# tqch/v-diffusion-torch

Measured on AMD Instinct MI355X. Metric: train_images_per_sec, higher is better.
Workload: dtype fp32 (bf16x3 split products in the tile-engine GEMMs)

## Files before the change

v-diffusion-torch_amd/csrc/norm.hip:

```cpp
#include "common.h"
#include <stdlib.h>

namespace {

constexpr int PPC = 128;

template <bool NT>
__device__ __forceinline__ f32x4 ld_stream(const float* p) {
    if (NT) return __builtin_nontemporal_load(reinterpret_cast<const f32x4*>(p));
    return *reinterpret_cast<const f32x4*>(p);
}
template <bool NT>
__device__ __forceinline__ void st_stream(float* p, f32x4 v) {
    if (NT) __builtin_nontemporal_store(v, reinterpret_cast<f32x4*>(p));
    else *reinterpret_cast<f32x4*>(p) = v;
}

struct ReduceArgs {
    const float* x; long long ldx;
    const float* dy; long long lddy;
    const float* coef;
    int act; float p_drop; unsigned long long seed; int resample; int has_norm;
    int H, W;
    long long HW;
    int C, nimg, chunks;
    float* part;
};

__device__ __forceinline__ f32x4 dz_finish(const ReduceArgs& p, f32x4 g, f32x4 xv, f32x4 sc, f32x4 of, unsigned long long vec_index) {
    if (p.p_drop > 0.f) g *= vd_dropout_scale4(p.seed, vec_index, p.p_drop);
    if (p.act) {
#pragma unroll
        for (int j = 0; j < 4; ++j) {
            const float z = xv[j] * sc[j] + of[j];
            const float s = vd_sigmoid(z);
            g[j] *= s * (1.f + z * (1.f - s));
        }
    }
    return g;
}

__device__ __forceinline__ f32x4 dz_of(const ReduceArgs& p, const float* dy_img, int pix, int c4, f32x4 xv, f32x4 sc,
                                       f32x4 of, unsigned long long vec_index) {
    f32x4 g;
    if (p.resample == VD_RS_NONE) {
        g = *reinterpret_cast<const f32x4*>(dy_img + (long long)pix * p.lddy + c4);
    } else {
        const int y = pix / p.W, x = pix - y * p.W;
        if (p.resample == VD_RS_DOWN) {
            const int Wo = p.W >> 1;
            g = *reinterpret_cast<const f32x4*>(dy_img + ((long long)(y >> 1) * Wo + (x >> 1)) * p.lddy + c4) * 0.25f;
        } else {
            const int Wo = p.W << 1;
            const float* b0 = dy_img + ((long long)(2 * y) * Wo + 2 * x) * p.lddy + c4;
            g = *reinterpret_cast<const f32x4*>(b0) + *reinterpret_cast<const f32x4*>(b0 + p.lddy) +
// ... 355 lines not shown
    const int c = (int)((long long)blockIdx.x - it[7]) * 16 + cx;
    float a = 0.f, bsum = 0.f;
    if (c < C)
        for (int b = ly; b < nimg; b += 16) { a += pgb[((long long)b * 2) * C + c]; bsum += pgb[((long long)b * 2 + 1) * C + c]; }
    sh[0][ly][cx] = a; sh[1][ly][cx] = bsum;
    __syncthreads();
    if (ly == 0 && c < C) {
        float s0 = 0.f, s1 = 0.f;
#pragma unroll
        for (int q = 0; q < 16; ++q) { s0 += sh[0][q][cx]; s1 += sh[1][q][cx]; }
        dgamma[c] = accumulate ? dgamma[c] + s0 : s0;
        dbeta[c] = accumulate ? dbeta[c] + s1 : s1;
    }
}

struct BwdApplyArgs {
    ReduceArgs r; const float* q; const float* add; long long ldadd; float* dx; long long lddx; int accumulate_dx;
};

__global__ __launch_bounds__(256) void gn_bwd_apply_kernel(const BwdApplyArgs a, int Cb) {
    const ReduceArgs& p = a.r;
    const int b = blockIdx.y, c0 = blockIdx.z * Cb;
    const int vecs = min(Cb, p.C - c0) >> 2, rows = 256 / vecs;
    const int r = threadIdx.x / vecs, c4 = c0 + 4 * (threadIdx.x % vecs);
    if (r >= rows) return;
    const int HW = (int)p.HW;
    const int p0 = blockIdx.x * APIX, np = min(APIX, HW - p0);
    f32x4 sc = {1.f, 1.f, 1.f, 1.f}, of = {0.f, 0.f, 0.f, 0.f}, nr = sc, nm = of;
    f32x4 q0 = sc, q1 = of, q2 = of;
    if (p.has_norm) {
        const float* cf = p.coef + (long long)b * 4 * p.C;
        sc = *reinterpret_cast<const f32x4*>(cf + c4);
        of = *reinterpret_cast<const f32x4*>(cf + p.C + c4);
        nr = *reinterpret_cast<const f32x4*>(cf + 2 * p.C + c4);
// ... 37 lines not shown
    for (int i = r; i < np; i += rows) {
        const int pix = p0 + i;
        f32x4 xv = {0.f, 0.f, 0.f, 0.f};
        if (p.has_norm) xv = *reinterpret_cast<const f32x4*>(ximg + (long long)pix * p.ldx + c4);
        const unsigned long long vi = ((unsigned long long)b * p.HW + pix) * vtot + (c4 >> 2);
        f32x4 d = dz_of(p, dimg, pix, c4, xv, sc, of, vi);
        if (p.has_norm) d = q0 * d - q1 - (xv * nr + nm) * q2;
        if (aimg) d += *reinterpret_cast<const f32x4*>(aimg + (long long)pix * a.ldadd + c4);
        float* o = oimg + (long long)pix * a.lddx + c4;
        if (a.accumulate_dx) d += *reinterpret_cast<const f32x4*>(o);
        *reinterpret_cast<f32x4*>(o) = d;
    }
}


struct FusedBwdArgs {
    BwdApplyArgs a; const float* gamma; const float* beta; const float* film; float* dfilm; float* pgb; int G, CS;
    int nsplit; float* xbuf; unsigned* cnt;
    unsigned* spin_max;
};

template <int NPT, int TPB, bool NT = false, bool SPLIT = false>
__global__ __launch_bounds__(TPB) void gn_bwd_fused_kernel(const FusedBwdArgs f) {
    __shared__ float red[TPB][8];
    __shared__ float chs[2][128];
    __shared__ float gm[2][32];
    constexpr int NREG = (NPT == 8 && TPB == 1024) ? 4 : NPT;
    __shared__ f32x4 xl[NPT - NREG > 0 ? NPT - NREG : 1][NPT - NREG > 0 ? TPB : 1];
    const ReduceArgs& p = f.a.r;
    const int CS = f.CS, C = p.C, tid = threadIdx.x;
    int b = blockIdx.y, slab = blockIdx.x, sib = 0, unit = 0;
    if (SPLIT) {
        const int lid = blockIdx.x, q = lid >> 3;
        sib = q % f.nsplit;
        unit = (q / f.nsplit) * 8 + (lid & 7);
        const int nslab = C / CS;
// ... 98 lines not shown
            }
            if (VD_PROBE_BUILD && f.spin_max) atomicMax(f.spin_max, spin);
        }
        __syncthreads();
        if (tid < 2 * CS) {
            const float* all = f.xbuf + (long long)unit * f.nsplit * 256 + (tid / CS) * 128 + (tid % CS);
            float t = 0.f;
            for (int k = 0; k < f.nsplit; ++k) t += __hip_atomic_load(all + k * 256, __ATOMIC_RELAXED, __HIP_MEMORY_SCOPE_AGENT);
            if (__hip_atomic_load(f.cnt + unit, __ATOMIC_RELAXED, __HIP_MEMORY_SCOPE_AGENT) >= (1u << 20)) t = __builtin_nanf("");
            chs[tid / CS][tid % CS] = t;
        }
        __syncthreads();
    }
    const int cg = C / f.G;
    if (tid < CS) {
        const int c = c0 + tid;
        const float s1 = chs[0][tid], s2 = chs[1][tid];
        float fs = 1.f;
        if (f.film) {
            fs = 1.f + f.film[(long long)b * 2 * C + C + c];
            if (sib == 0) {
                f.dfilm[(long long)b * 2 * C + c] = s1;
                f.dfilm[(long long)b * 2 * C + C + c] = f.gamma[c] * s2 + f.beta[c] * s1;
            }
        }
        const float k = f.gamma[c] * fs;
        if (sib == 0) {
            f.pgb[((long long)b * 2) * C + c] = fs * s2;
            f.pgb[((long long)b * 2 + 1) * C + c] = fs * s1;
        }
        chs[0][tid] = k * s1; chs[1][tid] = k * s2;
    }
    __syncthreads();
    if (tid < CS / cg) {
        float m1 = 0.f, m2 = 0.f;
        for (int c = tid * cg; c < (tid + 1) * cg; ++c) { m1 += chs[0][c]; m2 += chs[1][c]; }
        const float inv = 1.f / ((float)cg * (float)p.HW);
        gm[0][tid] = m1 * inv; gm[1][tid] = m2 * inv;
    }
    __syncthreads();
    if (!act) return;
    f32x4 q0, q1, q2;
#pragma unroll
    for (int j = 0; j < 4; ++j) {
        const int cl = 4 * v + j, c = c0 + cl, g = cl / cg;
        const float fs = f.film ? 1.f + f.film[(long long)b * 2 * C + C + c] : 1.f;
        q0[j] = nr[j] * f.gamma[c] * fs; q1[j] = nr[j] * gm[0][g]; q2[j] = nr[j] * gm[1][g];
    }
    const float* aimg = f.a.add ? f.a.add + ((long long)b * p.HW + pbeg) * f.a.ldadd : nullptr;
    float* oimg = f.a.dx + ((long long)b * p.HW + pbeg) * f.a.lddx;
#pragma unroll
    for (int i = 0; i < NPT; ++i) {
        const f32x4 xh = i < NREG ? xv[i < NREG ? i : 0] : xl[i < NREG ? 0 : i - NREG][tid];
        dz[i] = q0 * dz[i] - q1 - xh * q2;
    }
    if (aimg) {
        f32x4 ad[NPT];
#pragma unroll
        for (int i = 0; i < NPT; ++i) ad[i] = *reinterpret_cast<const f32x4*>(aimg + (long long)min(r + i * rows, HW - 1) * f.a.ldadd + c4);
#pragma unroll
        for (int i = 0; i < NPT; ++i) dz[i] += ad[i];
    }
    if (f.a.accumulate_dx) {
        f32x4 od[NPT];
#pragma unroll
        for (int i = 0; i < NPT; ++i) od[i] = *reinterpret_cast<const f32x4*>(oimg + (long long)min(r + i * rows, HW - 1) * f.a.lddx + c4);
#pragma unroll
        for (int i = 0; i < NPT; ++i) dz[i] += od[i];
    }
// ... 318 lines not shown
```

v-diffusion-torch_amd/csrc/wino43.hip:

```cpp
#include "common.h"
#include "../../include/vdiff_hip_dgrad_planes.h"
#include <stdlib.h>
#include <type_traits>

namespace {

typedef __attribute__((address_space(3))) void* lds_ptr_t;
constexpr unsigned OOB = 0x80000000u;
constexpr int KT = 8;
constexpr int TN = 32;
constexpr int TILES = 64;
constexpr int U_STAGE = 36 * 4 * 16 * 2 * 2;
constexpr int THREADS = 512;

struct Args43 {
    const float* x; long long ldx;
    const float* U;
    float* y; long long ldy;
    int nimg, H, W, K, N;
    int items_per_img;
    int ngrp;
    int ncb, nitems;
    const float* bias; const float* res; long long ldr;
    float* stats;
// ... 755 lines not shown
    o[0] = 1.265625f * v[0];
    o[1] = 1.6875f * q12 + 0.84375f * q34 + 1.265625f * v[5];
    o[2] = -2.8125f * v[0] - 2.25f * p12 - 0.5625f * p34;
    o[3] = -0.75f * q12 - 1.5f * q34 - 2.8125f * v[5];
    o[4] = v[0] + p12 + p34;
    o[5] = v[5];
}

struct In43 {
    const float* dV; long long plane;
    float* dx; long long lddx;
    int Cin;
};

template <int TW>
__global__ __launch_bounds__(256) void wino43_in_transpose_kernel(const In43 p) {
    constexpr int TPI = TW * TW, NQ = 256 / TPI;
    __shared__ f32x4 ring[12][256];
    const int tid = threadIdx.x, q = tid % NQ, tile = tid / NQ;
    const int ty = tile / TW, tx = tile - ty * TW;
    const int c4 = ((int)blockIdx.x * NQ + q) * 4;
    const bool in = c4 < p.Cin;
    f32x4 S[6][4];
    if (in) {
        const float* vp = p.dV + ((long long)blockIdx.y * TPI + tile) * p.Cin + c4;
#pragma unroll
        for (int a = 0; a < 6; ++a) {
            f32x4 v[6], r[6];
#pragma unroll
            for (int b = 0; b < 6; ++b) v[b] = *reinterpret_cast<const f32x4*>(vp + (long long)(6 * a + b) * p.plane);
            b6(v, r);
            ring[a][tid] = r[0]; ring[6 + a][tid] = r[5];
#pragma unroll
            for (int c = 0; c < 4; ++c) S[a][c] = r[c + 1];
        }
    }
    __syncthreads();
    if (in) {
        if (tx > 0) {
#pragma unroll
            for (int a = 0; a < 6; ++a) S[a][0] += ring[6 + a][tid - NQ];
        }
        if (tx < TW - 1) {
#pragma unroll
            for (int a = 0; a < 6; ++a) S[a][3] += ring[a][tid + NQ];
        }
    }
    __syncthreads();
    f32x4 P[4][4];
    if (in) {
#pragma unroll
        for (int c = 0; c < 4; ++c) {
            const f32x4 col[6] = {S[0][c], S[1][c], S[2][c], S[3][c], S[4][c], S[5][c]};
            f32x4 o[6];
            b6(col, o);
            ring[c][tid] = o[0]; ring[4 + c][tid] = o[5];
#pragma unroll
            for (int u = 0; u < 4; ++u) P[u][c] = o[u + 1];
        }
    }
    __syncthreads();
    if (!in) return;
    if (ty > 0) {
#pragma unroll
        for (int c = 0; c < 4; ++c) P[0][c] += ring[4 + c][tid - TW * NQ];
    }
    if (ty < TW - 1) {
#pragma unroll
        for (int c = 0; c < 4; ++c) P[3][c] += ring[c][tid + TW * NQ];
    }
    float* xp = p.dx + (((long long)blockIdx.y * (4 * TW) + 4 * ty) * (4 * TW) + 4 * tx) * p.lddx + c4;
#pragma unroll
    for (int u = 0; u < 4; ++u)
#pragma unroll
        for (int c = 0; c < 4; ++c) *reinterpret_cast<f32x4*>(xp + (long long)(u * 4 * TW + c) * p.lddx) = P[u][c];
}

struct Wg43Plan { bool ok; int T, S; size_t v_f, m_f, u_f, cs_f, gemm_bytes; };
Wg43Plan wg43_plan(int nimg, int H, int W, int Cin, int Cout) {
    Wg43Plan g = {};
    if (nimg <= 0 || H % 4 || W % 4 || H < 4 || W < 4 || Cin % 4 || Cout % 4) return g;
    g.T = nimg * (H / 4) * (W / 4);
    g.S = vd_gemm_grouped_wgrad_auto_split(36, Cout, Cin, g.T, (g.T + 1535) / 1536, 24);
    const size_t T16 = ((size_t)g.T + 15) / 16 * 16;
    g.v_f = (size_t)36 * T16 * Cin; g.m_f = (size_t)36 * T16 * Cout; g.u_f = (size_t)36 * Cout * Cin; g.cs_f = (size_t)36 * Cout;
    g.gemm_bytes = vd_gemm_grouped_wgrad_ws_bytes(36, Cout, Cin, g.S);
    g.ok = true;
    return g;
}

// ... 339 lines not shown
    return 1;
}

extern "C" size_t vd_conv3x3_wino43_dgrad_planes_ws_bytes(int32_t nimg, int32_t H, int32_t W, int32_t Cin, int32_t Cout) {
    const size_t T = (size_t)nimg * (H / 4) * (W / 4);
    return ((size_t)36 * Cout * Cin + (size_t)36 * T * Cin) * sizeof(float);
}

extern "C" int vd_conv3x3_dgrad_planes_preferred(int32_t nimg, int32_t H, int32_t W, int32_t Cin, int32_t Cout, int32_t training) {
    if (!training || !vd_conv3x3_wino43_dgrad_planes_supported(nimg, H, W, Cin, Cout, Cin)) return 0;
    static const long long floor_t = getenv("VD_PLANES_MIN_TILES") ? atoll(getenv("VD_PLANES_MIN_TILES")) : VD_PLANES_MIN_TILES;
    const long long T = (long long)nimg * (H / 4) * (W / 4);
    return T >= floor_t && Cin % 256 == 0 && Cout % 16 == 0;
}

extern "C" int vd_conv3x3_wino43_dgrad_planes(const float* dM, const float* w_oihw, float* dx, int64_t lddx, int32_t nimg, int32_t H, int32_t W,
                                              int32_t Cin, int32_t Cout, float* ws, size_t ws_bytes, int32_t phase, void* stream) {
    VD_REQUIRE(dM && w_oihw && dx && ws, "vd_conv3x3_wino43_dgrad_planes: null operand");
    VD_REQUIRE(vd_conv3x3_wino43_dgrad_planes_supported(nimg, H, W, Cin, Cout, lddx),
               "vd_conv3x3_wino43_dgrad_planes: unsupported geometry nimg=%d H=%d W=%d Cin=%d Cout=%d", nimg, H, W, Cin, Cout);
    VD_REQUIRE(vd_aligned16(dM) && vd_aligned16(dx) && vd_aligned16(ws), "vd_conv3x3_wino43_dgrad_planes: operands must be 16-byte aligned");
    VD_REQUIRE(ws_bytes >= vd_conv3x3_wino43_dgrad_planes_ws_bytes(nimg, H, W, Cin, Cout), "vd_conv3x3_wino43_dgrad_planes: workspace too small");
    VD_REQUIRE(phase == 7 || phase == 1 || phase == 2 || phase == 4, "vd_conv3x3_wino43_dgrad_planes: phase must be 7, 1, 2 or 4");
    const int TPI = (H / 4) * (W / 4), T = nimg * TPI;
    float* Ut = ws;
    float* dV = ws + (size_t)36 * Cout * Cin;
    hipStream_t st = (hipStream_t)stream;
    if (phase & 1) {
        const long long plane = (long long)Cout * Cin;
        hipLaunchKernelGGL(wino43_pack_planes_t_kernel, dim3((unsigned)((plane + 255) / 256)), dim3(256), 0, st, w_oihw, Ut, Cout, Cin);
        VD_LAUNCH_CHECK("wino43_pack_planes_t_kernel");
    }
    if (phase & 2) {
        vd_gemm_desc d = {};
        d.A = dM; d.B = Ut; d.C = dV;
        d.M = T; d.N = Cin; d.K = Cout; d.a_kind = VD_ROW; d.b_kind = VD_ROW;
        d.lda = Cout; d.ldb = Cout; d.ldc = Cin;
        d.batch = 36; d.nh = 1; d.alpha = 1.f;
        d.sAb = 16LL * Cout; d.sBb = (long long)Cout * Cin; d.sCb = (long long)T * Cin;
        const int rc = vd_gemm_rowblk(&d, 36LL * 16 * Cout, stream);
        if (rc) return rc;
    }
    if (phase & 4) {
        In43 o = {};
        o.dV = dV; o.plane = (long long)T * Cin; o.dx = dx; o.lddx = lddx; o.Cin = Cin;
        if (W == 32)
            hipLaunchKernelGGL(wino43_in_transpose_kernel<8>, dim3((unsigned)((Cin + 15) / 16), (unsigned)nimg), dim3(256), 0, st, o);
        else
            hipLaunchKernelGGL(wino43_in_transpose_kernel<4>, dim3((unsigned)((Cin + 63) / 64), (unsigned)nimg), dim3(256), 0, st, o);
        VD_LAUNCH_CHECK("wino43_in_transpose_kernel");
    }
    return 0;
}
```

v-diffusion-torch_amd/v_diffusion/_hip.py:

```python
import ctypes as C
import os
import re

import numpy as np
import torch

_HERE = os.path.dirname(os.path.abspath(__file__))
HEADER_PATH = os.path.join(os.path.dirname(os.path.dirname(_HERE)), "include", "vdiff_hip.h")
LIB_PATH = os.environ.get("VDIFF_HIP_LIB") or os.path.join(os.path.dirname(_HERE), "lib", "libvdiff_hip.so")

ROW, COL, IM2COL = 0, 1, 2
TILE_WIDE = 128256
RS_NONE, RS_DOWN, RS_UP = 0, 1, 2
OUT_TYPES = {"v": 0, "x0": 1, "eps": 2, "both": 3}
REWEIGHTS = {"constant": 0, "snr": 1, "snr_trunc": 2, "snr_1plus": 3}

_i32, _i64, _f32, _vp = C.c_int32, C.c_int64, C.c_float, C.c_void_p


class GemmDesc(C.Structure):
    _fields_ = [("A", _vp), ("B", _vp), ("C", _vp), ("bias", _vp), ("R", _vp),
                ("M", _i32), ("N", _i32), ("K", _i32), ("a_kind", _i32), ("b_kind", _i32),
                ("lda", _i64), ("ldb", _i64), ("ldc", _i64), ("ldr", _i64),
                ("batch", _i32), ("nh", _i32),
# ... 43 lines not shown
    if not os.path.exists(path):
        raise RuntimeError(f"{path} not found: the ctypes binding is read from the C headers of the source tree")
    with open(path) as f:
        tables = _parse_header(f.read())
    return [{name: _ctypes_of(name, *decl) for name, decl in t.items()} for t in tables]


_SIGNATURES, PROBE_EXPORTS = _header_signatures()
EXPORTS = tuple(_SIGNATURES)
EXT_HEADER_PATHS = (os.path.join(os.path.dirname(HEADER_PATH), "vdiff_hip_dgrad_planes.h"),)
_EXT_SIGNATURES = {name: sig for path in EXT_HEADER_PATHS for name, sig in _header_signatures(path)[0].items()}
EXT_EXPORTS = tuple(_EXT_SIGNATURES)
DPS_HEADER_PATHS = (os.path.join(os.path.dirname(HEADER_PATH), "vdiff_hip_dps.h"),)
_DPS_SIGNATURES = {name: sig for path in DPS_HEADER_PATHS for name, sig in _header_signatures(path)[0].items()}
DPS_EXPORTS = tuple(_DPS_SIGNATURES)

_lib = None


def lib():
    global _lib
    if _lib is None:
        if not os.path.exists(LIB_PATH):
            raise RuntimeError(
                f"{LIB_PATH} not found: build it with `python __graft_entry__.py` (or make -C v-diffusion-torch_amd/csrc). "
                "The v_diffusion hot path has no CPU/PyTorch fallback.")
        l = C.CDLL(LIB_PATH)
        for name, (res, args) in {**_SIGNATURES, **_EXT_SIGNATURES, **_DPS_SIGNATURES}.items():
            fn = getattr(l, name)
            fn.restype, fn.argtypes = res, args
        for name, (res, args) in PROBE_EXPORTS.items():
            if hasattr(l, name):
                fn = getattr(l, name)
                fn.restype, fn.argtypes = res, args
        _lib = l
    return _lib


class HipError(RuntimeError):
    pass


_CPU_TENSOR = "v_diffusion HIP op received a CPU tensor: the hot path runs on an MI355X only (no CPU fallback)"
# ... 344 lines not shown
def conv3x3_wino43_dgrad_planes(dm, w, dx, lddx, nimg, H, W, Cin, Cout):
    assert dm.numel() >= lib().vd_conv3x3_wino43_dm_floats(nimg, H, W, Cout) and w.is_contiguous() and tuple(w.shape) == (Cout, Cin, 3, 3)
    ws = workspace(lib().vd_conv3x3_wino43_dgrad_planes_ws_bytes(nimg, H, W, Cin, Cout), dm.device, "dgrad_planes")
    args = (ptr(dm), ptr(w), ptr(dx), lddx, nimg, H, W, Cin, Cout, ws.data_ptr(), ws.numel() * 4)
    phase = lambda ph: _check(lib().vd_conv3x3_wino43_dgrad_planes(*args, ph, stream()), "vd_conv3x3_wino43_dgrad_planes")
    if PROFILE is None:
        phase(7)
        return
    T = nimg * (H // 4) * (W // 4)
    with _TimedBytes("wino43_pack_planes_t_kernel", 4.0 * (9 + 36) * Cout * Cin):
        phase(1)
    with _TimedTile("gemm_dma_kernel<{tile}, 0, 0, false, {kt}>", 2.0 * 36 * T * Cout * Cin):
        phase(2)
    _note_bytes(PROFILE[-1][0], 4.0 * 36.0 * (T * (Cin + Cout) + Cout * Cin))
    with _TimedBytes("wino43_in_transpose_kernel", 4.0 * (36.0 * T * Cin + nimg * H * W * Cin)):
        phase(4)


def conv3x3_dgrad_wino43(dy, lddy, U43, dx, lddx, nimg, H, W, Cin, Cout):
    with _TimedName(f"wino43_conv_kernel<{W // 4}, false>", 2.0 * nimg * H * W * Cout * 9 * Cin):
        _check(lib().vd_conv3x3_dgrad_wino43(ptr(dy), lddy, ptr(U43), ptr(dx), lddx, nimg, H, W, Cin, Cout, stream()),
               "vd_conv3x3_dgrad_wino43")
    _note_bytes(f"wino43_conv_kernel<{W // 4}, false>", 4.0 * (nimg * H * W * (Cin + Cout) + 36 * Cout * Cin))


def conv3x3(x, ldx, wpack, bias, y, ldy, nimg, H, W, Cin, Cout, res=None, ldres=0, accumulate=False, stats_part=None):
    with _TimedTile("gemm_dma_kernel<{tile}, 2, 0, false, {kt}>", 2.0 * nimg * H * W * Cout * 9 * Cin):
        _check(lib().vd_conv3x3(ptr(x), ldx, ptr(wpack), ptr(bias), ptr(res), ldres, ptr(y), ldy, nimg, H, W, Cin, Cout,
                                int(accumulate), ptr(stats_part), stream()), "vd_conv3x3")

# ... 579 lines not shown
```

v-diffusion-torch_amd/v_diffusion/engine.py:

```python
import collections
import contextlib
import math

import torch

from . import _hip as H

GROUPS = 32
EPS = 1e-6
THIN = 8


def _ld(t):
    return t.stride(2)


def _chk(t):
    B, Hh, Ww, C = t.shape
    ld = t.stride(2)
    assert t.stride(3) == 1 and t.stride(1) == Ww * ld and t.stride(0) == Hh * Ww * ld, "not an NHWC view"
    return B, Hh, Ww, C, ld


def _splitk(M, N, K, n=1):
# ... 233 lines not shown
        if len(q) == H.GROUP_MAX:
            self._wgrad_flush_key(key)

    def _cwgrad(self, x, ldx, dy, lddy, *args, v=None, **kw):
        if v is not None:
            kw["v"] = v
        side = self._side
        if side is None:
            return H.conv3x3_wgrad(x, ldx, dy, lddy, *args, **kw)
        side.wait_stream(torch.cuda.current_stream())
        (x if v is None else v).record_stream(side)
        dy.record_stream(side)
        with torch.cuda.stream(side):
            H.conv3x3_wgrad(x, ldx, dy, lddy, *args, **kw)

    def _conv_bwd_planes(self, w, v, dy, lddy, dx, lddx, B, Hh, Ww, Cin, Cout, gw, gb):
        if v is None or not H.dgrad_planes_supported(B, Hh, Ww, Cin, Cout, lddy, lddx):
            return False
        dm = torch.empty(H.lib().vd_conv3x3_wino43_dm_floats(B, Hh, Ww, Cout), dtype=torch.float32, device=dy.device)
        H.conv3x3_wino43_dy_image(dy, lddy, B, Hh, Ww, Cout, dm)
        side = self._side
        if gw is None:
            pass
        elif side is None:
            H.conv3x3_wgrad_wino43_vm(v, dm, B, Hh, Ww, Cin, Cout, gw, Cin, Cout, dbias=gb)
        else:
            side.wait_stream(torch.cuda.current_stream())
            v.record_stream(side)
            dm.record_stream(side)
            with torch.cuda.stream(side):
                H.conv3x3_wgrad_wino43_vm(v, dm, B, Hh, Ww, Cin, Cout, gw, Cin, Cout, dbias=gb)
        H.conv3x3_wino43_dgrad_planes(dm, w, dx, lddx, B, Hh, Ww, Cin, Cout)
        return True

    def _side_join(self):
        if self._side is not None:
            torch.cuda.current_stream().wait_stream(self._side)

    def _wgrad_flush_key(self, key):
        q = self._wq.pop(key, None)
        if not q:
            return
        M, N, K, lda, ldb, ldc, _ = key
        ok = M % 4 == 0 and N % 4 == 0 and lda % 4 == 0 and ldb % 4 == 0 and max(lda, ldb, ldc) * 128 + 128 < 0x70000000 // 4 and \
            all(dy.data_ptr() % 16 == 0 and x.data_ptr() % 16 == 0 for dy, x, _, _ in q)
        if len(q) == 1 or not ok:
            for dy, x, dw, db in q:
# ... 282 lines not shown
                          ldres=_ld(sk), stats_part=pd, keep_v=v2)
        out_parts = self._parts(pd, Cout, Ho * Wo, rows)
        if tape is not None:
            tape[prefix] = dict(x=x, coef1=coef1, a1=None if v1 else a1, h1=h1, coef2=coef2, a2=None if v2 else a2, film=film,
                                xs=xs if has_skip else None, seed=seed, p=p_drop, v1=v1[0] if v1 else None, v2=v2[0] if v2 else None)
        return out_parts

    def _res_bwd(self, blk, ctx, dy, dx, dx_accumulate, ta, dfilms, G):
        mod = blk.res
        only_dx = G is None
        g = _NO_GRADS if only_dx else {s: G[name] for s, name in blk.res_names.items()}
        x, a1, h1, a2, film = ctx["x"], ctx["a1"], ctx["h1"], ctx["a2"], ctx["film"]
        B, Hh, Ww, Cin, ldx = _chk(x)
        _, Ho, Wo, Cout, lddy = _chk(dy)
        rs = blk.rs
        da2 = self._new(x, B, Ho, Wo, Cout)
        if not self._conv_bwd_planes(mod.conv2.weight, ctx["v2"], dy, lddy, da2, Cout, B, Ho, Wo, Cout, Cout, g["conv2.weight"], g["conv2.bias"]):
            if not only_dx:
                self._cwgrad(a2, Cout, dy, lddy, B, Ho, Wo, Cout, Cout, g["conv2.weight"], Cout, Cout, dbias=g["conv2.bias"], v=ctx["v2"])
            self._conv(dy, lddy, mod.conv2.weight, None, da2, Cout, B, Ho, Wo, Cout, Cout, dgrad=True)
        dh1 = self._new(x, B, Ho, Wo, Cout)
        c2, fi = blk.film
        dfilm = dfilms[c2][0 if only_dx else fi]
        H.gn_apply_bwd(da2, Cout, h1, Cout, ctx["coef2"], mod.norm2.weight, mod.norm2.bias, film, 1, ctx["p"], ctx["seed"],
                       H.RS_NONE, None, 0, dh1, Cout, False, dfilm, None, None, False, B, Ho, Wo, Cout, GROUPS,
                       pgb_keep=self._pgb(B, Cout, g["norm2.weight"], g["norm2.bias"]))
        del da2
        da1 = self._new(x, B, Ho, Wo, Cin)
        if not self._conv_bwd_planes(mod.conv1.weight, ctx["v1"], dh1, Cout, da1, Cin, B, Ho, Wo, Cin, Cout, g["conv1.weight"], g["conv1.bias"]):
            if not only_dx:
                self._cwgrad(a1, Cin, dh1, Cout, B, Ho, Wo, Cin, Cout, g["conv1.weight"], Cin, Cout, dbias=g["conv1.bias"], v=ctx["v1"])
            self._conv(dh1, Cout, mod.conv1.weight, None, da1, Cin, B, Ho, Wo, Cout, Cin, dgrad=True)
        del dh1
        if Cin != Cout:
            xs = ctx["xs"]
            P = B * Ho * Wo
            w = mod.skip.weight
            if not only_dx:
                self._wgrad(dy, xs, g["skip.weight"], g["skip.bias"], Cout, Cin, P, lddy, _ld(xs), Cin)
            dsk = self._new(x, B, Ho, Wo, Cin)
            H.gemm(dy, w, dsk, P, Cin, Cout, a_kind=H.ROW, b_kind=H.COL, lda=lddy, ldb=Cin, ldc=Cin)
        else:
            dsk = dy
        if rs != H.RS_NONE:
            addt = self._new(x, B, Hh, Ww, Cin)
            H.gn_apply_bwd(dsk, _ld(dsk), None, 0, None, None, None, None, 0, 0.0, 0, rs, None, 0, addt, Cin, False, None, None,
                           None, False, B, Hh, Ww, Cin, GROUPS)
        else:
            addt = dsk
        H.gn_apply_bwd(da1, Cin, x, ldx, ctx["coef1"], mod.norm1.weight, mod.norm1.bias, None, 1, 0.0, 0, rs, addt, _ld(addt),
                       dx, _ld(dx), dx_accumulate, None, None, None, False, B, Hh, Ww, Cin, GROUPS,
                       pgb_keep=self._pgb(B, Cin, g["norm1.weight"], g["norm1.bias"]))
        if not only_dx:
            self._linear_bwd(ta, mod.fc.weight, dfilm, g["fc.weight"], g["fc.bias"], None)

    def _attn_fwd(self, blk, x, dest, tape, x_parts=None):
        mod, prefix = blk.att, blk.att_prefix
        B, Hh, Ww, C, ldx = _chk(x)
        L, nh, hd = Hh * Ww, mod.num_heads, mod.head_dim
        hid = nh * hd
        xn = self._new(x, B, Hh, Ww, C)
        coef = self._norm(x, x_parts, mod.norm, None, 0, 0.0, 0, H.RS_NONE, xn, B, Hh, Ww, C)
        qkv = self._new(x, B, L, 3 * hid)
        H.gemm(xn, mod.proj_in.weight, qkv, B * L, 3 * hid, C, a_kind=H.ROW, b_kind=H.ROW, lda=C, ldb=C, ldc=3 * hid,
               bias=mod.proj_in.bias)
        ld = 3 * hid
        alpha = 1.0 / math.sqrt(hd)
# ... 343 lines not shown
```

Measured before the change: 2314.

## Fuse GroupNorm backward into Winograd dgrad input-transform epilogue

Adds a variant of the Winograd 4x3 dgrad input-transpose kernel that applies the GroupNorm/SiLU/dropout backward in-register. Each block holds a whole image for its channel slice, so it does the per-channel and per-group reductions and writes dx directly, plus the add and accumulate. This removes the intermediate da tensor write/read and the separate gn_apply_bwd launch for the resblock convolutions. The cost is heavier register and LDS use in the transpose kernel and reduced parallelism, since one block must cover all pixels of an image; it only applies for some shapes.

New measurement: 2351, median of 5. No clear change (+1.6%).

```diff
diff --git a/include/vdiff_hip_dgrad_gn.h b/include/vdiff_hip_dgrad_gn.h
--- /dev/null
+++ b/include/vdiff_hip_dgrad_gn.h
@@ -0,0 +1,21 @@
+#ifndef VDIFF_HIP_DGRAD_GN_H
+#define VDIFF_HIP_DGRAD_GN_H
+#include <stddef.h>
+#include <stdint.h>
+
+#ifdef __cplusplus
+extern "C" {
+#endif
+
+int vd_conv3x3_wino43_dgrad_planes_gn_supported(int32_t nimg, int32_t H, int32_t W, int32_t Cin, int32_t Cout, int64_t ldx, int64_t ldadd,
+                                                int64_t lddx, int32_t G, int32_t resample);
+int vd_conv3x3_wino43_dgrad_planes_gn(const float* dM, const float* w_oihw, int32_t nimg, int32_t H, int32_t W, int32_t Cin, int32_t Cout,
+                                      float* ws, size_t ws_bytes, int32_t phase, const float* x, int64_t ldx, const float* coef,
+                                      const float* gamma, const float* beta, const float* film, int32_t act, float p_drop, uint64_t seed,
+                                      int32_t resample, const float* add, int64_t ldadd, float* dx, int64_t lddx, int32_t accumulate_dx,
+                                      float* dfilm, float* pgb_keep, int32_t G, void* stream);
+
+#ifdef __cplusplus
+}
+#endif
+#endif
diff --git a/v-diffusion-torch_amd/csrc/gn_bwd.h b/v-diffusion-torch_amd/csrc/gn_bwd.h
--- /dev/null
+++ b/v-diffusion-torch_amd/csrc/gn_bwd.h
@@ -0,0 +1,84 @@
+#ifndef VD_GN_BWD_H
+#define VD_GN_BWD_H
+#include "common.h"
+
+namespace {
+
+template <bool NT>
+__device__ __forceinline__ f32x4 ld_stream(const float* p) {
+    if (NT) return __builtin_nontemporal_load(reinterpret_cast<const f32x4*>(p));
+    return *reinterpret_cast<const f32x4*>(p);
+}
+template <bool NT>
+__device__ __forceinline__ void st_stream(float* p, f32x4 v) {
+    if (NT) __builtin_nontemporal_store(v, reinterpret_cast<f32x4*>(p));
+    else *reinterpret_cast<f32x4*>(p) = v;
+}
+
+struct ReduceArgs {
+    const float* x; long long ldx;
+    const float* dy; long long lddy;
+    const float* coef;
+    int act; float p_drop; unsigned long long seed; int resample; int has_norm;
+    int H, W;
+    long long HW;
+    int C, nimg, chunks;
+    float* part;
+};
+
+struct BwdApplyArgs {
+    ReduceArgs r; const float* q; const float* add; long long ldadd; float* dx; long long lddx; int accumulate_dx;
+};
+
+struct FusedBwdArgs {
+    BwdApplyArgs a; const float* gamma; const float* beta; const float* film; float* dfilm; float* pgb; int G, CS;
+    int nsplit; float* xbuf; unsigned* cnt;
+    unsigned* spin_max;
+};
+
+__device__ __forceinline__ f32x4 dz_finish(const ReduceArgs& p, f32x4 g, f32x4 xv, f32x4 sc, f32x4 of, unsigned long long vec_index) {
+    if (p.p_drop > 0.f) g *= vd_dropout_scale4(p.seed, vec_index, p.p_drop);
+    if (p.act) {
+#pragma unroll
+        for (int j = 0; j < 4; ++j) {
+            const float z = xv[j] * sc[j] + of[j];
+            const float s = vd_sigmoid(z);
+            g[j] *= s * (1.f + z * (1.f - s));
+        }
+    }
+    return g;
+}
+
+__device__ __forceinline__ void gn_bwd_channel(const FusedBwdArgs& f, int b, int c, float s1, float s2, bool write, float& ks1, float& ks2) {
+    const int C = f.a.r.C;
+    float fs = 1.f;
+    if (f.film) {
+        fs = 1.f + f.film[(long long)b * 2 * C + C + c];
+        if (write) {
+            f.dfilm[(long long)b * 2 * C + c] = s1;
+            f.dfilm[(long long)b * 2 * C + C + c] = f.gamma[c] * s2 + f.beta[c] * s1;
+        }
+    }
+    const float k = f.gamma[c] * fs;
+    if (write) {
+        f.pgb[((long long)b * 2) * C + c] = fs * s2;
+        f.pgb[((long long)b * 2 + 1) * C + c] = fs * s1;
+    }
+    ks1 = k * s1; ks2 = k * s2;
+}
+
+__device__ __forceinline__ void gn_bwd_q(const FusedBwdArgs& f, int b, int c0, int cl, int cg, f32x4 nr, const float* gm1, const float* gm2,
+                                         f32x4& q0, f32x4& q1, f32x4& q2) {
+    const int C = f.a.r.C;
+#pragma unroll
+    for (int j = 0; j < 4; ++j) {
+        const int c = c0 + cl + j, g = (cl + j) / cg;
+        const float fs = f.film ? 1.f + f.film[(long long)b * 2 * C + C + c] : 1.f;
+        q0[j] = nr[j] * f.gamma[c] * fs; q1[j] = nr[j] * gm1[g]; q2[j] = nr[j] * gm2[g];
+    }
+}
+
+__device__ __forceinline__ f32x4 gn_bwd_dx(f32x4 q0, f32x4 q1, f32x4 q2, f32x4 dz, f32x4 xh) { return q0 * dz - q1 - xh * q2; }
+
+}
+#endif
diff --git a/v-diffusion-torch_amd/csrc/norm.hip b/v-diffusion-torch_amd/csrc/norm.hip
--- a/v-diffusion-torch_amd/csrc/norm.hip
+++ b/v-diffusion-torch_amd/csrc/norm.hip
@@ -1,44 +1,10 @@
 #include "common.h"
+#include "gn_bwd.h"
 #include <stdlib.h>
 
 namespace {
 
 constexpr int PPC = 128;
-
-template <bool NT>
-__device__ __forceinline__ f32x4 ld_stream(const float* p) {
-    if (NT) return __builtin_nontemporal_load(reinterpret_cast<const f32x4*>(p));
-    return *reinterpret_cast<const f32x4*>(p);
-}
-template <bool NT>
-__device__ __forceinline__ void st_stream(float* p, f32x4 v) {
-    if (NT) __builtin_nontemporal_store(v, reinterpret_cast<f32x4*>(p));
-    else *reinterpret_cast<f32x4*>(p) = v;
-}
-
-struct ReduceArgs {
-    const float* x; long long ldx;
-    const float* dy; long long lddy;
-    const float* coef;
-    int act; float p_drop; unsigned long long seed; int resample; int has_norm;
-    int H, W;
-    long long HW;
-    int C, nimg, chunks;
-    float* part;
-};
-
-__device__ __forceinline__ f32x4 dz_finish(const ReduceArgs& p, f32x4 g, f32x4 xv, f32x4 sc, f32x4 of, unsigned long long vec_index) {
-    if (p.p_drop > 0.f) g *= vd_dropout_scale4(p.seed, vec_index, p.p_drop);
-    if (p.act) {
-#pragma unroll
-        for (int j = 0; j < 4; ++j) {
-            const float z = xv[j] * sc[j] + of[j];
-            const float s = vd_sigmoid(z);
-            g[j] *= s * (1.f + z * (1.f - s));
-        }
-    }
-    return g;
-}
 
 __device__ __forceinline__ f32x4 dz_of(const ReduceArgs& p, const float* dy_img, int pix, int c4, f32x4 xv, f32x4 sc,
                                        f32x4 of, unsigned long long vec_index) {
@@ -424,10 +390,6 @@
     }
 }
 
-struct BwdApplyArgs {
-    ReduceArgs r; const float* q; const float* add; long long ldadd; float* dx; long long lddx; int accumulate_dx;
-};
-
 __global__ __launch_bounds__(256) void gn_bwd_apply_kernel(const BwdApplyArgs a, int Cb) {
     const ReduceArgs& p = a.r;
     const int b = blockIdx.y, c0 = blockIdx.z * Cb;
@@ -495,12 +457,6 @@
 }
 
 
-struct FusedBwdArgs {
-    BwdApplyArgs a; const float* gamma; const float* beta; const float* film; float* dfilm; float* pgb; int G, CS;
-    int nsplit; float* xbuf; unsigned* cnt;
-    unsigned* spin_max;
-};
-
 template <int NPT, int TPB, bool NT = false, bool SPLIT = false>
 __global__ __launch_bounds__(TPB) void gn_bwd_fused_kernel(const FusedBwdArgs f) {
     __shared__ float red[TPB][8];
@@ -629,22 +585,9 @@
     }
     const int cg = C / f.G;
     if (tid < CS) {
-        const int c = c0 + tid;
-        const float s1 = chs[0][tid], s2 = chs[1][tid];
-        float fs = 1.f;
-        if (f.film) {
-            fs = 1.f + f.film[(long long)b * 2 * C + C + c];
-            if (sib == 0) {
-                f.dfilm[(long long)b * 2 * C + c] = s1;
-                f.dfilm[(long long)b * 2 * C + C + c] = f.gamma[c] * s2 + f.beta[c] * s1;
-            }
-        }
-        const float k = f.gamma[c] * fs;
-        if (sib == 0) {
-            f.pgb[((long long)b * 2) * C + c] = fs * s2;
-            f.pgb[((long long)b * 2 + 1) * C + c] = fs * s1;
-        }
-        chs[0][tid] = k * s1; chs[1][tid] = k * s2;
+        float ks1, ks2;
+        gn_bwd_channel(f, b, c0 + tid, chs[0][tid], chs[1][tid], sib == 0, ks1, ks2);
+        chs[0][tid] = ks1; chs[1][tid] = ks2;
     }
     __syncthreads();
     if (tid < CS / cg) {
@@ -656,18 +599,13 @@
     __syncthreads();
     if (!act) return;
     f32x4 q0, q1, q2;
-#pragma unroll
-    for (int j = 0; j < 4; ++j) {
-        const int cl = 4 * v + j, c = c0 + cl, g = cl / cg;
-        const float fs = f.film ? 1.f + f.film[(long long)b * 2 * C + C + c] : 1.f;
-        q0[j] = nr[j] * f.gamma[c] * fs; q1[j] = nr[j] * gm[0][g]; q2[j] = nr[j] * gm[1][g];
-    }
+    gn_bwd_q(f, b, c0, 4 * v, cg, nr, gm[0], gm[1], q0, q1, q2);
     const float* aimg = f.a.add ? f.a.add + ((long long)b * p.HW + pbeg) * f.a.ldadd : nullptr;
     float* oimg = f.a.dx + ((long long)b * p.HW + pbeg) * f.a.lddx;
 #pragma unroll
     for (int i = 0; i < NPT; ++i) {
         const f32x4 xh = i < NREG ? xv[i < NREG ? i : 0] : xl[i < NREG ? 0 : i - NREG][tid];
-        dz[i] = q0 * dz[i] - q1 - xh * q2;
+        dz[i] = gn_bwd_dx(q0, q1, q2, dz[i], xh);
     }
     if (aimg) {
         f32x4 ad[NPT];
diff --git a/v-diffusion-torch_amd/csrc/wino43.hip b/v-diffusion-torch_amd/csrc/wino43.hip
--- a/v-diffusion-torch_amd/csrc/wino43.hip
+++ b/v-diffusion-torch_amd/csrc/wino43.hip
@@ -1,5 +1,7 @@
 #include "common.h"
+#include "gn_bwd.h"
 #include "../../include/vdiff_hip_dgrad_planes.h"
+#include "../../include/vdiff_hip_dgrad_gn.h"
 #include <stdlib.h>
 #include <type_traits>
 
@@ -793,9 +795,8 @@
 };
 
 template <int TW>
-__global__ __launch_bounds__(256) void wino43_in_transpose_kernel(const In43 p) {
+__device__ __forceinline__ void in_transpose_tiles(const In43& p, f32x4 (&ring)[12][256], f32x4 (&P)[4][4]) {
     constexpr int TPI = TW * TW, NQ = 256 / TPI;
-    __shared__ f32x4 ring[12][256];
     const int tid = threadIdx.x, q = tid % NQ, tile = tid / NQ;
     const int ty = tile / TW, tx = tile - ty * TW;
     const int c4 = ((int)blockIdx.x * NQ + q) * 4;
@@ -826,7 +827,6 @@
         }
     }
     __syncthreads();
-    f32x4 P[4][4];
     if (in) {
 #pragma unroll
         for (int c = 0; c < 4; ++c) {
@@ -848,11 +848,122 @@
 #pragma unroll
         for (int c = 0; c < 4; ++c) P[3][c] += ring[c][tid + TW * NQ];
     }
+}
+
+template <int TW>
+__global__ __launch_bounds__(256) void wino43_in_transpose_kernel(const In43 p) {
+    constexpr int TPI = TW * TW, NQ = 256 / TPI;
+    __shared__ f32x4 ring[12][256];
+    const int tid = threadIdx.x, q = tid % NQ, tile = tid / NQ;
+    const int ty = tile / TW, tx = tile - ty * TW;
+    const int c4 = ((int)blockIdx.x * NQ + q) * 4;
+    f32x4 P[4][4];
+    in_transpose_tiles<TW>(p, ring, P);
+    if (c4 >= p.Cin) return;
     float* xp = p.dx + (((long long)blockIdx.y * (4 * TW) + 4 * ty) * (4 * TW) + 4 * tx) * p.lddx + c4;
 #pragma unroll
     for (int u = 0; u < 4; ++u)
 #pragma unroll
         for (int c = 0; c < 4; ++c) *reinterpret_cast<f32x4*>(xp + (long long)(u * 4 * TW + c) * p.lddx) = P[u][c];
+}
+
+template <int TW>
+__global__ __launch_bounds__(256) void wino43_in_transpose_gn_kernel(const In43 p, const FusedBwdArgs f) {
+    constexpr int TPI = TW * TW, NQ = 256 / TPI, CS = 4 * NQ, W = 4 * TW, HW = W * W;
+    constexpr bool NT = CS % 32 == 0;
+    __shared__ f32x4 ring[12][256];
+    const ReduceArgs& r = f.a.r;
+    const int tid = threadIdx.x, q = tid % NQ, tile = tid / NQ;
+    const int ty = tile / TW, tx = tile - ty * TW;
+    const int b = blockIdx.y, c0 = (int)blockIdx.x * CS, c4 = c0 + 4 * q, C = p.Cin;
+    const bool in = c4 < C;
+    f32x4 P[4][4];
+    in_transpose_tiles<TW>(p, ring, P);
+    const long long pix0 = (long long)b * HW + (4 * ty) * W + 4 * tx;
+    f32x4 xh[4][4];
+    f32x4 a0 = {0.f, 0.f, 0.f, 0.f}, a1 = a0, nr = a0;
+    if (in) {
+        const float* cf = r.coef + (long long)b * 4 * C;
+        const f32x4 sc = *reinterpret_cast<const f32x4*>(cf + c4), of = *reinterpret_cast<const f32x4*>(cf + C + c4);
+        const f32x4 nm = *reinterpret_cast<const f32x4*>(cf + 3 * C + c4);
+        nr = *reinterpret_cast<const f32x4*>(cf + 2 * C + c4);
+        const float* xp = r.x + pix0 * r.ldx + c4;
+#pragma unroll
+        for (int u = 0; u < 4; ++u)
+#pragma unroll
+            for (int c = 0; c < 4; ++c) xh[u][c] = ld_stream<NT>(xp + (long long)(u * W + c) * r.ldx);
+        const unsigned long long vtot = C >> 2;
+#pragma unroll
+        for (int u = 0; u < 4; ++u)
+#pragma unroll
+            for (int c = 0; c < 4; ++c) {
+                const unsigned long long vi = ((unsigned long long)pix0 + u * W + c) * vtot + (c4 >> 2);
+                P[u][c] = dz_finish(r, P[u][c], xh[u][c], sc, of, vi);
+                xh[u][c] = xh[u][c] * nr + nm;
+                a0 += P[u][c];
+                a1 += P[u][c] * xh[u][c];
+            }
+    }
+    __syncthreads();
+    float* red = reinterpret_cast<float*>(&ring[0][0]);
+    float* lvl = red + 2048;
+    float* chs = lvl + 256;
+    float* gm = chs + 128;
+#pragma unroll
+    for (int j = 0; j < 4; ++j) { red[tid * 8 + j] = a0[j]; red[tid * 8 + 4 + j] = a1[j]; }
+    __syncthreads();
+    constexpr int comps = NQ * 8, fan = 256 / comps, per = TPI / fan;
+    {
+        const int pair = tid / fan, k = tid - pair * fan, qq = pair >> 3, jj = pair & 7;
+        float part = 0.f;
+#pragma unroll
+        for (int t = k * per; t < (k + 1) * per; ++t) part += red[(t * NQ + qq) * 8 + jj];
+        lvl[tid] = part;
+    }
+    __syncthreads();
+    if (tid < comps) {
+        float s = 0.f;
+#pragma unroll
+        for (int k = 0; k < fan; ++k) s += lvl[tid * fan + k];
+        const int qq = tid >> 3, jj = tid & 7;
+        chs[(jj >> 2) * 64 + qq * 4 + (jj & 3)] = s;
+    }
+    __syncthreads();
+    const int cg = C / f.G;
+    if (tid < CS) {
+        float ks1 = 0.f, ks2 = 0.f;
+        if (c0 + tid < C) gn_bwd_channel(f, b, c0 + tid, chs[tid], chs[64 + tid], true, ks1, ks2);
+        chs[tid] = ks1; chs[64 + tid] = ks2;
+    }
+    __syncthreads();
+    if (tid < CS / cg) {
+        float m1 = 0.f, m2 = 0.f;
+        for (int c = tid * cg; c < (tid + 1) * cg; ++c) { m1 += chs[c]; m2 += chs[64 + c]; }
+        const float inv = 1.f / ((float)cg * (float)HW);
+        gm[tid] = m1 * inv; gm[64 + tid] = m2 * inv;
+    }
+    __syncthreads();
+    if (!in) return;
+    f32x4 q0, q1, q2;
+    gn_bwd_q(f, b, c0, 4 * q, cg, nr, gm, gm + 64, q0, q1, q2);
+    const float* ap = f.a.add ? f.a.add + pix0 * f.a.ldadd + c4 : nullptr;
+    float* op = f.a.dx + pix0 * f.a.lddx + c4;
+#pragma unroll
+    for (int u = 0; u < 4; ++u) {
+        f32x4 d[4];
+#pragma unroll
+        for (int c = 0; c < 4; ++c) d[c] = gn_bwd_dx(q0, q1, q2, P[u][c], xh[u][c]);
+        if (ap) {
+#pragma unroll
+            for (int c = 0; c < 4; ++c) d[c] += *reinterpret_cast<const f32x4*>(ap + (long long)(u * W + c) * f.a.ldadd);
+        }
+        if (f.a.accumulate_dx) {
+#pragma unroll
+            for (int c = 0; c < 4; ++c) d[c] += *reinterpret_cast<const f32x4*>(op + (long long)(u * W + c) * f.a.lddx);
+        }
+#pragma unroll
+        for (int c = 0; c < 4; ++c) st_stream<NT>(op + (long long)(u * W + c) * f.a.lddx, d[c]);
+    }
 }
 
 struct Wg43Plan { bool ok; int T, S; size_t v_f, m_f, u_f, cs_f, gemm_bytes; };
@@ -1222,6 +1333,9 @@
     return T >= floor_t && Cin % 256 == 0 && Cout % 16 == 0;
 }
 
+static int dgrad_planes_front(const float* dM, const float* w_oihw, int32_t nimg, int32_t H, int32_t W, int32_t Cin, int32_t Cout, float* ws,
+                              int32_t phase, void* stream);
+
 extern "C" int vd_conv3x3_wino43_dgrad_planes(const float* dM, const float* w_oihw, float* dx, int64_t lddx, int32_t nimg, int32_t H, int32_t W,
                                               int32_t Cin, int32_t Cout, float* ws, size_t ws_bytes, int32_t phase, void* stream) {
     VD_REQUIRE(dM && w_oihw && dx && ws, "vd_conv3x3_wino43_dgrad_planes: null operand");
@@ -1230,6 +1344,69 @@
     VD_REQUIRE(vd_aligned16(dM) && vd_aligned16(dx) && vd_aligned16(ws), "vd_conv3x3_wino43_dgrad_planes: operands must be 16-byte aligned");
     VD_REQUIRE(ws_bytes >= vd_conv3x3_wino43_dgrad_planes_ws_bytes(nimg, H, W, Cin, Cout), "vd_conv3x3_wino43_dgrad_planes: workspace too small");
     VD_REQUIRE(phase == 7 || phase == 1 || phase == 2 || phase == 4, "vd_conv3x3_wino43_dgrad_planes: phase must be 7, 1, 2 or 4");
+    const int rc = dgrad_planes_front(dM, w_oihw, nimg, H, W, Cin, Cout, ws, phase, stream);
+    if (rc) return rc;
+    if (phase & 4) {
+        In43 o = {};
+        o.dV = ws + (size_t)36 * Cout * Cin; o.plane = (long long)nimg * (H / 4) * (W / 4) * Cin; o.dx = dx; o.lddx = lddx; o.Cin = Cin;
+        hipStream_t st = (hipStream_t)stream;
+        if (W == 32)
+            hipLaunchKernelGGL(wino43_in_transpose_kernel<8>, dim3((unsigned)((Cin + 15) / 16), (unsigned)nimg), dim3(256), 0, st, o);
+        else
+            hipLaunchKernelGGL(wino43_in_transpose_kernel<4>, dim3((unsigned)((Cin + 63) / 64), (unsigned)nimg), dim3(256), 0, st, o);
+        VD_LAUNCH_CHECK("wino43_in_transpose_kernel");
+    }
+    return 0;
+}
+
+extern "C" int vd_conv3x3_wino43_dgrad_planes_gn_supported(int32_t nimg, int32_t H, int32_t W, int32_t Cin, int32_t Cout, int64_t ldx,
+                                                           int64_t ldadd, int64_t lddx, int32_t G, int32_t resample) {
+    if (!vd_conv3x3_wino43_dgrad_planes_supported(nimg, H, W, Cin, Cout, lddx)) return 0;
+    if (resample != VD_RS_NONE || G <= 0 || Cin % G) return 0;
+    if ((W == 32 ? 16 : 64) % (Cin / G)) return 0;
+    if (ldx % 4 || ldx < Cin || ldadd % 4 || (ldadd != 0 && ldadd < Cin)) return 0;
+    return 1;
+}
+
+extern "C" int vd_conv3x3_wino43_dgrad_planes_gn(const float* dM, const float* w_oihw, int32_t nimg, int32_t H, int32_t W, int32_t Cin,
+                                                 int32_t Cout, float* ws, size_t ws_bytes, int32_t phase, const float* x, int64_t ldx,
+                                                 const float* coef, const float* gamma, const float* beta, const float* film, int32_t act,
+                                                 float p_drop, uint64_t seed, int32_t resample, const float* add, int64_t ldadd, float* dx,
+                                                 int64_t lddx, int32_t accumulate_dx, float* dfilm, float* pgb_keep, int32_t G, void* stream) {
+    VD_REQUIRE(dM && w_oihw && dx && ws, "vd_conv3x3_wino43_dgrad_planes_gn: null operand");
+    VD_REQUIRE(x && coef && gamma && beta && pgb_keep,
+               "vd_conv3x3_wino43_dgrad_planes_gn: needs a norm (x, coef, gamma, beta) and the [nimg][2][Cin] buffer for its per-image dgamma / dbeta terms");
+    VD_REQUIRE(!film || dfilm, "vd_conv3x3_wino43_dgrad_planes_gn: film given without dfilm");
+    VD_REQUIRE(vd_conv3x3_wino43_dgrad_planes_gn_supported(nimg, H, W, Cin, Cout, ldx, add ? ldadd : 0, lddx, G, resample),
+               "vd_conv3x3_wino43_dgrad_planes_gn: unsupported geometry nimg=%d H=%d W=%d Cin=%d Cout=%d G=%d resample=%d", nimg, H, W, Cin, Cout,
+               G, resample);
+    VD_REQUIRE(vd_aligned16(dM) && vd_aligned16(ws) && vd_aligned16(x) && vd_aligned16(coef) && vd_aligned16(add) && vd_aligned16(dx),
+               "vd_conv3x3_wino43_dgrad_planes_gn: operands must be 16-byte aligned");
+    VD_REQUIRE(ws_bytes >= vd_conv3x3_wino43_dgrad_planes_ws_bytes(nimg, H, W, Cin, Cout), "vd_conv3x3_wino43_dgrad_planes_gn: workspace too small");
+    VD_REQUIRE(phase == 7 || phase == 1 || phase == 2 || phase == 4, "vd_conv3x3_wino43_dgrad_planes_gn: phase must be 7, 1, 2 or 4");
+    const int rc = dgrad_planes_front(dM, w_oihw, nimg, H, W, Cin, Cout, ws, phase, stream);
+    if (rc) return rc;
+    if (phase & 4) {
+        In43 o = {};
+        o.dV = ws + (size_t)36 * Cout * Cin; o.plane = (long long)nimg * (H / 4) * (W / 4) * Cin; o.Cin = Cin;
+        FusedBwdArgs f = {};
+        ReduceArgs& p = f.a.r;
+        p.x = x; p.ldx = ldx; p.coef = coef; p.act = act; p.p_drop = p_drop; p.seed = seed; p.resample = VD_RS_NONE; p.has_norm = 1;
+        p.H = H; p.W = W; p.HW = (long long)H * W; p.C = Cin; p.nimg = nimg;
+        f.a.add = add; f.a.ldadd = ldadd; f.a.dx = dx; f.a.lddx = lddx; f.a.accumulate_dx = accumulate_dx;
+        f.gamma = gamma; f.beta = beta; f.film = film; f.dfilm = dfilm; f.pgb = pgb_keep; f.G = G; f.CS = W == 32 ? 16 : 64; f.nsplit = 1;
+        hipStream_t st = (hipStream_t)stream;
+        if (W == 32)
+            hipLaunchKernelGGL(wino43_in_transpose_gn_kernel<8>, dim3((unsigned)((Cin + 15) / 16), (unsigned)nimg), dim3(256), 0, st, o, f);
+        else
+            hipLaunchKernelGGL(wino43_in_transpose_gn_kernel<4>, dim3((unsigned)((Cin + 63) / 64), (unsigned)nimg), dim3(256), 0, st, o, f);
+        VD_LAUNCH_CHECK("wino43_in_transpose_gn_kernel");
+    }
+    return 0;
+}
+
+static int dgrad_planes_front(const float* dM, const float* w_oihw, int32_t nimg, int32_t H, int32_t W, int32_t Cin, int32_t Cout, float* ws,
+                              int32_t phase, void* stream) {
     const int TPI = (H / 4) * (W / 4), T = nimg * TPI;
     float* Ut = ws;
     float* dV = ws + (size_t)36 * Cout * Cin;
@@ -1249,14 +1426,5 @@
         const int rc = vd_gemm_rowblk(&d, 36LL * 16 * Cout, stream);
         if (rc) return rc;
     }
-    if (phase & 4) {
-        In43 o = {};
-        o.dV = dV; o.plane = (long long)T * Cin; o.dx = dx; o.lddx = lddx; o.Cin = Cin;
-        if (W == 32)
-            hipLaunchKernelGGL(wino43_in_transpose_kernel<8>, dim3((unsigned)((Cin + 15) / 16), (unsigned)nimg), dim3(256), 0, st, o);
-        else
-            hipLaunchKernelGGL(wino43_in_transpose_kernel<4>, dim3((unsigned)((Cin + 63) / 64), (unsigned)nimg), dim3(256), 0, st, o);
-        VD_LAUNCH_CHECK("wino43_in_transpose_kernel");
-    }
     return 0;
 }
diff --git a/v-diffusion-torch_amd/v_diffusion/_hip.py b/v-diffusion-torch_amd/v_diffusion/_hip.py
--- a/v-diffusion-torch_amd/v_diffusion/_hip.py
+++ b/v-diffusion-torch_amd/v_diffusion/_hip.py
@@ -81,6 +81,9 @@
 DPS_HEADER_PATHS = (os.path.join(os.path.dirname(HEADER_PATH), "vdiff_hip_dps.h"),)
 _DPS_SIGNATURES = {name: sig for path in DPS_HEADER_PATHS for name, sig in _header_signatures(path)[0].items()}
 DPS_EXPORTS = tuple(_DPS_SIGNATURES)
+DGRAD_GN_HEADER_PATHS = (os.path.join(os.path.dirname(HEADER_PATH), "vdiff_hip_dgrad_gn.h"),)
+_DGRAD_GN_SIGNATURES = {name: sig for path in DGRAD_GN_HEADER_PATHS for name, sig in _header_signatures(path)[0].items()}
+DGRAD_GN_EXPORTS = tuple(_DGRAD_GN_SIGNATURES)
 
 _lib = None
 
@@ -93,7 +96,7 @@
                 f"{LIB_PATH} not found: build it with `python __graft_entry__.py` (or make -C v-diffusion-torch_amd/csrc). "
                 "The v_diffusion hot path has no CPU/PyTorch fallback.")
         l = C.CDLL(LIB_PATH)
-        for name, (res, args) in {**_SIGNATURES, **_EXT_SIGNATURES, **_DPS_SIGNATURES}.items():
+        for name, (res, args) in {**_SIGNATURES, **_EXT_SIGNATURES, **_DPS_SIGNATURES, **_DGRAD_GN_SIGNATURES}.items():
             fn = getattr(l, name)
             fn.restype, fn.argtypes = res, args
         for name, (res, args) in PROBE_EXPORTS.items():
@@ -468,6 +471,34 @@
         phase(2)
     _note_bytes(PROFILE[-1][0], 4.0 * 36.0 * (T * (Cin + Cout) + Cout * Cin))
     with _TimedBytes("wino43_in_transpose_kernel", 4.0 * (36.0 * T * Cin + nimg * H * W * Cin)):
+        phase(4)
+
+
+DGRAD_GN = os.environ.get("VD_DGRAD_GN", "1")
+
+
+def dgrad_planes_gn_supported(nimg, H, W, Cin, Cout, ldx, ldadd, lddx, G, resample):
+    return DGRAD_GN != "0" and bool(lib().vd_conv3x3_wino43_dgrad_planes_gn_supported(nimg, H, W, Cin, Cout, ldx, ldadd, lddx, G, resample))
+
+
+def conv3x3_wino43_dgrad_planes_gn(dm, w, nimg, H, W, Cin, Cout, x, ldx, coef, gamma, beta, film, act, p_drop, seed, add, ldadd, dx, lddx,
+                                   accumulate_dx, dfilm, pgb_keep, G=32):
+    assert dm.numel() >= lib().vd_conv3x3_wino43_dm_floats(nimg, H, W, Cout) and w.is_contiguous() and tuple(w.shape) == (Cout, Cin, 3, 3)
+    ws = workspace(lib().vd_conv3x3_wino43_dgrad_planes_ws_bytes(nimg, H, W, Cin, Cout), dm.device, "dgrad_planes")
+    head = (ptr(dm), ptr(w), nimg, H, W, Cin, Cout, ws.data_ptr(), ws.numel() * 4)
+    tail = (ptr(x), ldx, ptr(coef), ptr(gamma), ptr(beta), ptr(film), int(act), float(p_drop), int(seed), RS_NONE, ptr(add), ldadd, ptr(dx),
+            lddx, int(accumulate_dx), ptr(dfilm), ptr(pgb_keep), G)
+    phase = lambda ph: _check(lib().vd_conv3x3_wino43_dgrad_planes_gn(*head, ph, *tail, stream()), "vd_conv3x3_wino43_dgrad_planes_gn")
+    if PROFILE is None:
+        phase(7)
+        return
+    T = nimg * (H // 4) * (W // 4)
+    with _TimedBytes("wino43_pack_planes_t_kernel", 4.0 * (9 + 36) * Cout * Cin):
+        phase(1)
+    with _TimedTile("gemm_dma_kernel<{tile}, 0, 0, false, {kt}>", 2.0 * 36 * T * Cout * Cin):
+        phase(2)
+    _note_bytes(PROFILE[-1][0], 4.0 * 36.0 * (T * (Cin + Cout) + Cout * Cin))
+    with _TimedBytes("wino43_in_transpose_gn_kernel", 4.0 * (36.0 * T * Cin + nimg * H * W * Cin * (2 + (add is not None) + bool(accumulate_dx)))):
         phase(4)
 
 
diff --git a/v-diffusion-torch_amd/v_diffusion/engine.py b/v-diffusion-torch_amd/v_diffusion/engine.py
--- a/v-diffusion-torch_amd/v_diffusion/engine.py
+++ b/v-diffusion-torch_amd/v_diffusion/engine.py
@@ -271,8 +271,14 @@
         with torch.cuda.stream(side):
             H.conv3x3_wgrad(x, ldx, dy, lddy, *args, **kw)
 
-    def _conv_bwd_planes(self, w, v, dy, lddy, dx, lddx, B, Hh, Ww, Cin, Cout, gw, gb):
+    @staticmethod
+    def _planes_gn(v, B, Hh, Ww, Cin, Cout, lddy, ldx, ldadd, lddx, rs=H.RS_NONE):
+        return v is not None and H.dgrad_planes_supported(B, Hh, Ww, Cin, Cout, lddy, Cin) and \
+            H.dgrad_planes_gn_supported(B, Hh, Ww, Cin, Cout, ldx, ldadd, lddx, GROUPS, rs)
+
+    def _conv_bwd_planes(self, w, v, dy, lddy, dx, lddx, B, Hh, Ww, Cin, Cout, gw, gb, gn=None):
         if v is None or not H.dgrad_planes_supported(B, Hh, Ww, Cin, Cout, lddy, lddx):
+            assert gn is None
             return False
         dm = torch.empty(H.lib().vd_conv3x3_wino43_dm_floats(B, Hh, Ww, Cout), dtype=torch.float32, device=dy.device)
         H.conv3x3_wino43_dy_image(dy, lddy, B, Hh, Ww, Cout, dm)
@@ -287,7 +293,10 @@
             dm.record_stream(side)
             with torch.cuda.stream(side):
                 H.conv3x3_wgrad_wino43_vm(v, dm, B, Hh, Ww, Cin, Cout, gw, Cin, Cout, dbias=gb)
-        H.conv3x3_wino43_dgrad_planes(dm, w, dx, lddx, B, Hh, Ww, Cin, Cout)
+        if gn is None:
+            H.conv3x3_wino43_dgrad_planes(dm, w, dx, lddx, B, Hh, Ww, Cin, Cout)
+        else:
+            H.conv3x3_wino43_dgrad_planes_gn(dm, w, B, Hh, Ww, Cin, Cout, *gn)
         return True
 
     def _side_join(self):
@@ -600,24 +609,31 @@
         B, Hh, Ww, Cin, ldx = _chk(x)
         _, Ho, Wo, Cout, lddy = _chk(dy)
         rs = blk.rs
-        da2 = self._new(x, B, Ho, Wo, Cout)
-        if not self._conv_bwd_planes(mod.conv2.weight, ctx["v2"], dy, lddy, da2, Cout, B, Ho, Wo, Cout, Cout, g["conv2.weight"], g["conv2.bias"]):
-            if not only_dx:
-                self._cwgrad(a2, Cout, dy, lddy, B, Ho, Wo, Cout, Cout, g["conv2.weight"], Cout, Cout, dbias=g["conv2.bias"], v=ctx["v2"])
-            self._conv(dy, lddy, mod.conv2.weight, None, da2, Cout, B, Ho, Wo, Cout, Cout, dgrad=True)
         dh1 = self._new(x, B, Ho, Wo, Cout)
         c2, fi = blk.film
         dfilm = dfilms[c2][0 if only_dx else fi]
-        H.gn_apply_bwd(da2, Cout, h1, Cout, ctx["coef2"], mod.norm2.weight, mod.norm2.bias, film, 1, ctx["p"], ctx["seed"],
-                       H.RS_NONE, None, 0, dh1, Cout, False, dfilm, None, None, False, B, Ho, Wo, Cout, GROUPS,
-                       pgb_keep=self._pgb(B, Cout, g["norm2.weight"], g["norm2.bias"]))
-        del da2
-        da1 = self._new(x, B, Ho, Wo, Cin)
-        if not self._conv_bwd_planes(mod.conv1.weight, ctx["v1"], dh1, Cout, da1, Cin, B, Ho, Wo, Cin, Cout, g["conv1.weight"], g["conv1.bias"]):
-            if not only_dx:
-                self._cwgrad(a1, Cin, dh1, Cout, B, Ho, Wo, Cin, Cout, g["conv1.weight"], Cin, Cout, dbias=g["conv1.bias"], v=ctx["v1"])
-            self._conv(dh1, Cout, mod.conv1.weight, None, da1, Cin, B, Ho, Wo, Cout, Cin, dgrad=True)
-        del dh1
+        if self._planes_gn(ctx["v2"], B, Ho, Wo, Cout, Cout, lddy, Cout, 0, Cout):
+            self._conv_bwd_planes(mod.conv2.weight, ctx["v2"], dy, lddy, None, Cout, B, Ho, Wo, Cout, Cout, g["conv2.weight"], g["conv2.bias"],
+                                  gn=(h1, Cout, ctx["coef2"], mod.norm2.weight, mod.norm2.bias, film, 1, ctx["p"], ctx["seed"], None, 0, dh1,
+                                      Cout, False, dfilm, self._pgb(B, Cout, g["norm2.weight"], g["norm2.bias"]), GROUPS))
+        else:
+            da2 = self._new(x, B, Ho, Wo, Cout)
+            if not self._conv_bwd_planes(mod.conv2.weight, ctx["v2"], dy, lddy, da2, Cout, B, Ho, Wo, Cout, Cout, g["conv2.weight"], g["conv2.bias"]):
+                if not only_dx:
+                    self._cwgrad(a2, Cout, dy, lddy, B, Ho, Wo, Cout, Cout, g["conv2.weight"], Cout, Cout, dbias=g["conv2.bias"], v=ctx["v2"])
+                self._conv(dy, lddy, mod.conv2.weight, None, da2, Cout, B, Ho, Wo, Cout, Cout, dgrad=True)
+            H.gn_apply_bwd(da2, Cout, h1, Cout, ctx["coef2"], mod.norm2.weight, mod.norm2.bias, film, 1, ctx["p"], ctx["seed"],
+                           H.RS_NONE, None, 0, dh1, Cout, False, dfilm, None, None, False, B, Ho, Wo, Cout, GROUPS,
+                           pgb_keep=self._pgb(B, Cout, g["norm2.weight"], g["norm2.bias"]))
+            del da2
+        fuse1 = rs == H.RS_NONE and self._planes_gn(ctx["v1"], B, Ho, Wo, Cin, Cout, Cout, ldx, lddy if Cin == Cout else Cin, _ld(dx))
+        if not fuse1:
+            da1 = self._new(x, B, Ho, Wo, Cin)
+            if not self._conv_bwd_planes(mod.conv1.weight, ctx["v1"], dh1, Cout, da1, Cin, B, Ho, Wo, Cin, Cout, g["conv1.weight"], g["conv1.bias"]):
+                if not only_dx:
+                    self._cwgrad(a1, Cin, dh1, Cout, B, Ho, Wo, Cin, Cout, g["conv1.weight"], Cin, Cout, dbias=g["conv1.bias"], v=ctx["v1"])
+                self._conv(dh1, Cout, mod.conv1.weight, None, da1, Cin, B, Ho, Wo, Cout, Cin, dgrad=True)
+            del dh1
         if Cin != Cout:
             xs = ctx["xs"]
             P = B * Ho * Wo
@@ -634,9 +650,15 @@
                            None, False, B, Hh, Ww, Cin, GROUPS)
         else:
             addt = dsk
-        H.gn_apply_bwd(da1, Cin, x, ldx, ctx["coef1"], mod.norm1.weight, mod.norm1.bias, None, 1, 0.0, 0, rs, addt, _ld(addt),
-                       dx, _ld(dx), dx_accumulate, None, None, None, False, B, Hh, Ww, Cin, GROUPS,
-                       pgb_keep=self._pgb(B, Cin, g["norm1.weight"], g["norm1.bias"]))
+        if fuse1:
+            self._conv_bwd_planes(mod.conv1.weight, ctx["v1"], dh1, Cout, None, Cin, B, Ho, Wo, Cin, Cout, g["conv1.weight"], g["conv1.bias"],
+                                  gn=(x, ldx, ctx["coef1"], mod.norm1.weight, mod.norm1.bias, None, 1, 0.0, 0, addt, _ld(addt), dx, _ld(dx),
+                                      dx_accumulate, None, self._pgb(B, Cin, g["norm1.weight"], g["norm1.bias"]), GROUPS))
+            del dh1
+        else:
+            H.gn_apply_bwd(da1, Cin, x, ldx, ctx["coef1"], mod.norm1.weight, mod.norm1.bias, None, 1, 0.0, 0, rs, addt, _ld(addt),
+                           dx, _ld(dx), dx_accumulate, None, None, None, False, B, Hh, Ww, Cin, GROUPS,
+                           pgb_keep=self._pgb(B, Cin, g["norm1.weight"], g["norm1.bias"]))
         if not only_dx:
             self._linear_bwd(ta, mod.fc.weight, dfilm, g["fc.weight"], g["fc.bias"], None)
 
```
